# gpuopenanalytics/libgdf

Hardware: AMD Instinct MI355X
Metric: hash-join probe rows/s (higher is better)
Workload: dtype int64

## Files before the change

libgdf_amd/csrc/internal.h:

```cpp
#pragma once
#include "common.h"
#include "lab.h"
#include "prof.h"

namespace gdf_amd {

hipError_t read_back(void *host_dst, const void *dev_src, size_t bytes);
struct ReadTicket { bool pending = false; int lane = 0; size_t bytes = 0; const void *dev_src = nullptr; };
hipError_t read_back_begin(ReadTicket *t, const void *dev_src, size_t bytes, int lane);
hipError_t read_back_end(ReadTicket *t, void *host_dst);

void place_budget_begin();
bool place_budget_left();
int place_draws_now(int max_draws);
struct PlaceRound {
  double t0;
  PlaceRound();
  ~PlaceRound();
};

int device_cu_count();

gdf_error scan_u32(const uint32_t *in, uint32_t *out, size_t n, bool inclusive);
gdf_error scan_u64(const uint64_t *in, uint64_t *out, size_t n, bool inclusive);
gdf_error scan_u32_async(const uint32_t *in, uint32_t *out, size_t n, bool inclusive, DevBuf *scratch);

gdf_error order_rows(const KeyTable &t, uint32_t n, DevBuf &perm, DevBuf *sorted_keys, bool *keys_exact, size_t *perm64 = nullptr,
                     bool *perm64_written = nullptr);
gdf_error key_ranges(const KeyTable &t, long long *lo_hi, int windows = 1, int64_t window_rows = 0);
gdf_error radix_sort_pairs_u64(uint64_t *&kin, uint64_t *&kout, uint64_t *&vin, uint64_t *&vout, uint32_t n, uint64_t varying);
gdf_error radix_sort_pairs_k32_u64(uint32_t *&kin, uint32_t *&kout, uint64_t *&vin, uint64_t *&vout, uint32_t n, uint64_t varying);
gdf_error group_by_sort(int ncols, gdf_column **cols, gdf_column *col_agg, gdf_column *out_col_indices,
                        gdf_column **out_col_values, gdf_column *out_col_agg, gdf_context *ctxt, int op);

}
```

libgdf_amd/csrc/join.hip:

```cpp
#include "internal.h"
#include "launch.h"
#include "gdf/gdf_amd_ext.h"

#include <cmath>
#include <cstdio>

#include <algorithm>
#include <cstdlib>
#include <deque>
#include <memory>
#include <type_traits>
#include <vector>

namespace gdf_amd {

enum KeyMode : int { KM_RAW_INT = 0, KM_RAW_FLOAT, KM_PACKED, KM_HASHED };

struct KeyPlan {
  int mode;
  int verify;
  int narrow;
  uint64_t kmin;
  uint64_t kspan;
  uint64_t klimit;
// ... 1120 lines not shown
  const T incl = wave_scan_incl(v);
  block_sync();
  if (lane_id() == WAVE - 1) lds_wave[threadIdx.x / WAVE] = incl;
  block_sync();
  T woff = 0, tot = 0;
#pragma unroll
  for (int w = 0; w < JK_BK_THREADS / WAVE; ++w) {
    if (w < (int)(threadIdx.x / WAVE)) woff += lds_wave[w];
    tot += lds_wave[w];
  }
  *total = tot;
  return woff + incl - v;
}
constexpr uint32_t JK_L2MAP_LDS_SEGS = 16384;
__global__ __launch_bounds__(JK_BK_THREADS) void jk_make_l2map(const uint32_t *__restrict__ fill, uint32_t nseg, uint32_t cap1, uint32_t tile,
                                                               uint32_t *__restrict__ seg_begin, uint32_t *__restrict__ seg_end,
                                                               uint32_t *__restrict__ tile_prefix, uint32_t *__restrict__ ntiles,
                                                               uint32_t fj_world, uint32_t ncoarse, const uint32_t *__restrict__ rstart = nullptr,
                                                               const uint32_t *__restrict__ rcap = nullptr) {
  __shared__ uint32_t lds_wave[JK_BK_THREADS / WAVE];
  extern __shared__ __attribute__((aligned(16))) uint32_t l2map_lds[];
  const uint32_t per = (nseg + JK_BK_THREADS - 1) / JK_BK_THREADS;
  const uint32_t c0 = threadIdx.x * per;
  auto region_of = [&](uint32_t seg) -> uint32_t {
    if (!fj_world) return seg;
    const uint32_t cs = seg >> 3, c = cs / fj_world, sender = cs - c * fj_world;
    return ((sender * ncoarse + c) << 3) | (seg & 7u);
  };
  auto filled = [&](uint32_t region) -> uint32_t { const uint32_t n = fill[region], room = rcap ? rcap[region] : cap1; return n < room ? n : room; };
  const bool pow2 = (tile & (tile - 1u)) == 0;
  const int shift = __ffs((int)tile) - 1;
  auto tiles_of = [&](uint32_t n) -> uint32_t { return pow2 ? (n + tile - 1u) >> shift : (n + tile - 1u) / tile; };
  if (nseg <= JK_L2MAP_LDS_SEGS) {
    constexpr int MAXK = (int)(JK_L2MAP_LDS_SEGS / JK_BK_THREADS);
    uint32_t n_[MAXK], first_[MAXK];
#pragma unroll
    for (int k = 0; k < MAXK; ++k) {
      const uint32_t c = (uint32_t)k * JK_BK_THREADS + threadIdx.x;
      n_[k] = 0; first_[k] = 0;
      if (c < nseg) {
        const uint32_t r = region_of(c);
        n_[k] = filled(r);
        first_[k] = rstart ? rstart[r] : r * cap1;
        l2map_lds[c] = tiles_of(n_[k]);
      }
    }
    block_sync();
    uint32_t mine = 0;
    for (uint32_t c = c0; c < c0 + per && c < nseg; ++c) mine += l2map_lds[c];
    uint32_t total;
    uint32_t run = bk_block_scan<uint32_t>(mine, lds_wave, &total);
    for (uint32_t c = c0; c < c0 + per && c < nseg; ++c) { const uint32_t t = l2map_lds[c]; l2map_lds[c] = run; run += t; }
    block_sync();
#pragma unroll
    for (int k = 0; k < MAXK; ++k) {
      const uint32_t c = (uint32_t)k * JK_BK_THREADS + threadIdx.x;
      if (c < nseg) { seg_begin[c] = first_[k]; seg_end[c] = first_[k] + n_[k]; tile_prefix[c] = l2map_lds[c]; }
    }
    if (threadIdx.x == 0) { tile_prefix[nseg] = total; *ntiles = total; }
    return;
  }
  uint32_t mine = 0;
  for (uint32_t c = c0; c < c0 + per && c < nseg; ++c) mine += tiles_of(filled(region_of(c)));
  uint32_t total;
  uint32_t run = bk_block_scan<uint32_t>(mine, lds_wave, &total);
  for (uint32_t c = c0; c < c0 + per && c < nseg; ++c) {
    const uint32_t r = region_of(c), n = filled(r);
    const uint32_t first = rstart ? rstart[r] : r * cap1;
    seg_begin[c] = first;
    seg_end[c] = first + n;
    tile_prefix[c] = run;
    run += tiles_of(n);
  }
  if (threadIdx.x == 0) { tile_prefix[nseg] = total; *ntiles = total; }
}
static gdf_error l2map_prepare(uint32_t nseg, size_t *lds) {
  *lds = nseg <= JK_L2MAP_LDS_SEGS ? sizeof(uint32_t) * (size_t)nseg : 0;
  return allow_lds(jk_make_l2map, sizeof(uint32_t) * JK_L2MAP_LDS_SEGS);
}
__global__ __launch_bounds__(256) void jk_init_cursor(uint32_t *cur, uint32_t nfine, uint32_t cap2, const uint32_t *__restrict__ fstart = nullptr) {
  for (uint32_t f = blockIdx.x * 256 + threadIdx.x; f <= nfine; f += gridDim.x * 256) cur[f] = f < nfine ? (fstart ? fstart[f] : f * cap2) : 0u;
}

__global__ __launch_bounds__(JK_BK_THREADS) void jk_level2_index(const uint32_t *__restrict__ begin, const uint32_t *__restrict__ cnt, uint32_t nfine, int b2,
                                                                 uint32_t tile, uint32_t *__restrict__ coarse_off, uint32_t *__restrict__ tile_prefix,
                                                                 uint32_t *__restrict__ cursor) {
  __shared__ uint32_t lds_wave[JK_BK_THREADS / WAVE];
  const uint32_t ncoarse = nfine >> b2, total_rows = begin[nfine - 1] + cnt[nfine - 1];
  uint32_t run = 0;
  for (uint32_t base = 0; base < ncoarse; base += JK_BK_THREADS) {
    const uint32_t c = base + threadIdx.x;
    uint32_t first = 0, tiles = 0;
    if (c < ncoarse) {
      first = begin[(size_t)c << b2];
      const uint32_t next = c + 1 < ncoarse ? begin[(size_t)(c + 1) << b2] : total_rows;
      tiles = (next - first + tile - 1) / tile;
    }
    uint32_t total;
    const uint32_t before = bk_block_scan<uint32_t>(tiles, lds_wave, &total);
    if (c < ncoarse) { coarse_off[c] = first; tile_prefix[c] = run + before; }
    run += total;
    block_sync();
  }
  if (threadIdx.x == 0) { coarse_off[ncoarse] = total_rows; tile_prefix[ncoarse] = run; }
  for (uint32_t f = threadIdx.x; f < nfine; f += JK_BK_THREADS) cursor[f] = begin[f];
}

struct Unit {
  uint32_t build_begin, build_count;
  uint32_t probe_begin, probe_count;
};

__global__ __launch_bounds__(256) void jk_make_units(uint32_t nfine, uint32_t cap2, const uint32_t *__restrict__ cursor,
                                                     const uint32_t *__restrict__ level1_flag,
                                                     const uint32_t *__restrict__ build_begin, const uint32_t *__restrict__ build_cnt,
                                                     int keep_probe, Unit *__restrict__ units, uint64_t *__restrict__ off,
                                                     unsigned long long *__restrict__ state, const uint32_t *__restrict__ fstart = nullptr,
                                                     const uint32_t *__restrict__ fcap = nullptr) {
  const uint32_t f = blockIdx.x * 256 + threadIdx.x;
  const uint32_t fc = f < nfine ? f : nfine - 1;
  const uint32_t cur = cursor[fc], bn = build_cnt[fc], bb = build_begin[fc];
  const uint32_t first = fstart ? fstart[fc] : fc * cap2;
  if (fcap) cap2 = fcap[fc];
  const uint32_t grown = f < nfine ? cur - first : 0u;
  const uint32_t all = grown < cap2 ? grown : cap2;
  const uint32_t pn = (all != 0 && (bn != 0 || keep_probe)) ? all : 0u;
  const uint32_t nun = (pn + JK_PROBE_CHUNK - 1) / JK_PROBE_CHUNK;
  const uint32_t incl_u = wave_scan_incl(nun);
  const unsigned long long incl_t = wave_scan_incl((unsigned long long)pn);
  const unsigned long long sum_all = wave_reduce_add((unsigned long long)all);
  unsigned long long base_u = 0, base_t = 0;
  if (lane_id() == WAVE - 1) {
    if (incl_u) { base_u = atomicAdd(&state[0], (unsigned long long)incl_u); base_t = atomicAdd(&state[1], incl_t); }
    if (sum_all) atomicAdd(&state[2], sum_all);
  }
  base_u = __shfl(base_u, WAVE - 1, WAVE);
  base_t = __shfl(base_t, WAVE - 1, WAVE);
  unsigned long long u = base_u + incl_u - nun, o = base_t + incl_t - pn;
  for (uint32_t at = 0; at < pn; at += JK_PROBE_CHUNK) {
    const uint32_t cnt = pn - at < JK_PROBE_CHUNK ? pn - at : JK_PROBE_CHUNK;
    units[u] = Unit{bb, bn, first + at, cnt};
    off[u] = o;
    ++u;
    o += cnt;
  }
  if (f == 0) state[3] = (unsigned long long)((cursor[nfine] ? 1u : 0u) | ((level1_flag && *level1_flag) ? 2u : 0u));
}

struct ProbeArgs {
  Tuples build, probe;
  const Unit *units;
  uint32_t nslots;
  uint32_t cap;
  int keep_unmatched_probe;
  int verify;
  uint8_t *build_matched;
  uint64_t *counts;
  int32_t *out_probe; int32_t *out_build;
  int unused;
  uint64_t kbias;
  int optimistic;
  unsigned long long *opt_state;
  uint32_t *unit_todo;
  uint32_t sample_n;
  const unsigned long long *nunits_dev;
  uint32_t *unit_pairs;
  int pay_mode;
  const void *pay_src[2];
  void *pay_out[2];
  int key_width;
  const void *key_src;
  void *key_out;
  int bpay_mode;
  const void *bpay_src[2];
  void *bpay_out[2];
  int p6_fb;
  uint32_t p6_world;
  uint64_t p6_kbias;
};
__device__ __forceinline__ void pay_gather(const ProbeArgs &a, unsigned long long pos, int32_t prow) {
  if (a.pay_mode == 1 || a.pay_mode == 4) {
    ((uint64_t *)a.pay_out[0])[pos] = ((const uint64_t *)a.pay_src[0])[prow];
    if (a.pay_mode == 4) ((uint64_t *)a.pay_out[1])[pos] = ((const uint64_t *)a.pay_src[1])[prow];
  } else if (a.pay_mode) {
    ((uint32_t *)a.pay_out[0])[pos] = ((const uint32_t *)a.pay_src[0])[prow];
    if (a.pay_mode == 3) ((uint32_t *)a.pay_out[1])[pos] = ((const uint32_t *)a.pay_src[1])[prow];
  }
  if (a.key_width == 8) ((uint64_t *)a.key_out)[pos] = ((const uint64_t *)a.key_src)[prow];
// ... 1351 lines not shown
    } else {
      const size_t lds = sizeof(TileLds<true, 1024>);
      GDF_TRY(with_int<8, 4>(fast, [&](auto F) {
        return with_bools([&](auto M) {
          return launch_lds("jk_scatter1", jk_scatter1<F(), true, 1024, M(), true>, dim3(g.nchunks), dim3(1024), lds, t, plan, g, H1off, out);
        }, masked);
      }));
    }
    HIP_CHECK_LAST();
    return GDF_SUCCESS;
  }
  if (masked) {
    if (fast == 4) return launch_scatter1_n<4, true, true>(t, plan, g, H1off, out);
    return narrow ? launch_scatter1_n<8, true, true>(t, plan, g, H1off, out)
                  : launch_scatter1_n<8, false, true>(t, plan, g, H1off, out);
  }
  if (fast == 4) return launch_scatter1_n<4, true, false>(t, plan, g, H1off, out);
  if (fast == 8) return narrow ? launch_scatter1_n<8, true, false>(t, plan, g, H1off, out)
                               : launch_scatter1_n<8, false, false>(t, plan, g, H1off, out);
  return narrow ? launch_scatter1_n<0, true, false>(t, plan, g, H1off, out)
                : launch_scatter1_n<0, false, false>(t, plan, g, H1off, out);
}
static int fast_key_width(const KeyTable &t, const KeyPlan &plan) {
  if (t.ncols != 1 || (plan.mode != KM_RAW_INT && plan.mode != KM_RAW_FLOAT) || t.nrows < 2) return 0;
  if (t.col[0].valid && t.nrows < 64) return 0;
  if (t.col[0].width == 8) return 8;
  if (t.col[0].width == 4 && plan.narrow && plan.kmin == 0) return 4;
  return 0;
}
template <bool NARROW, int THREADS>
static constexpr size_t level2_lds_bytes() { using Tile = TileLds<NARROW, THREADS>; return offsetof(Tile, cursor); }
static gdf_error launch_scatter2(bool narrow, uint32_t ntiles, const PartGeom &g, Level2Map m, Tuples in,
                                 uint32_t *cursor, Tuples out, bool p6 = false, bool in6 = false, int pw = 1) {
  if (in6 && !(p6 && !m.keys32 && g.b1 == 8)) return GDF_INVALID_API_CALL;
  if (!in6 && p6 && !narrow && m.keys32) return GDF_INVALID_API_CALL;
  m.ntiles = ntiles;
  m.xcd_order = (ntiles >= 64 && !lab::path_on("GDF_JK_NO_XCD_ORDER")) ? 1 : 0;
  const uint32_t grid = sc2_grid(m, ntiles);
  auto launch = [&](const char *name, auto kernel, int threads, size_t lds) -> gdf_error {
    GDF_TRY(launch_lds(name, kernel, dim3(grid), dim3(threads), lds, g, m, in, cursor, out));
    HIP_CHECK_LAST();
    return GDF_SUCCESS;
  };
  if (in6) {
    if (!narrow)
      return launch("jk_scatter2_w10", jk_scatter2<false, 256, 0, true, false, true>, 256, level2_lds_bytes<false, 256>());
    return launch("jk_scatter2", jk_scatter2<true, 256, 0, true, false, true>, 256, sizeof(TileLds<true, 256>));
  }
  if (p6 && !narrow)
    return launch("jk_scatter2_w10", jk_scatter2<false, 256, 0, true>, 256, level2_lds_bytes<false, 256>());
  if (p6 || m.keys32) {
    const size_t lds = sizeof(TileLds<true, 256>);
    if (p6 && m.keys32) return launch("jk_scatter2", jk_scatter2<true, 256, 0, true, true>, 256, lds);
    if (p6) return launch("jk_scatter2", jk_scatter2<true, 256, 0, true, false>, 256, lds);
    return launch("jk_scatter2", jk_scatter2<true, 256, 0, false, true>, 256, lds);
  }
  if (narrow && in.pay && pw == 2) {
    using Tile = TileLds<true, 256, 2, JK_PAY_ITEMS>;
    return launch("jk_scatter2", jk_scatter2<true, 256, 2>, 256, offsetof(Tile, cursor));
  }
  if (narrow && in.pay)
    return launch("jk_scatter2", jk_scatter2<true, 256, 1>, 256, sizeof(TileLds<true, 256, true, JK_PAY_ITEMS>));
  if (narrow) return launch("jk_scatter2", jk_scatter2<true, JK_SC2_THREADS>, JK_SC2_THREADS, sizeof(TileLds<true, JK_SC2_THREADS>));
  return launch("jk_scatter2", jk_scatter2<false, JK_SC2_THREADS>, JK_SC2_THREADS, sizeof(TileLds<false, JK_SC2_THREADS>));
}

static gdf_error launch_scatter1_pay(int fast, int pmode, const KeyTable &t, const KeyPlan &plan, const PartGeom &g, const uint32_t *H1off,
                                     const PaySrc &ps, Tuples out) {
  GDF_TRY(with_int<8, 4>(fast, [&](auto F) {
    return with_int<1, 2, 3, 4>(pmode, [&](auto M) {
      const size_t lds = sizeof(TileLds<true, JK_PAY_THREADS, pay_words(M()), pay_items1(M())>);
      return launch_lds("jk_scatter1", jk_scatter1_pay<F(), M()>, dim3(g.nchunks), dim3(JK_PAY_THREADS), lds, t, plan, g, H1off, ps, out);
    });
  }));
  HIP_CHECK_LAST();
  return GDF_SUCCESS;
}

static gdf_error partition_side(const KeyTable &t, KeyPlan &plan, PartGeom g, SideBufs *sb, bool decide_narrow, const PaySrc *pay = nullptr,
                                int pmode = 0, bool device_index = false, bool want_p6 = false, bool keep_running = false) {
  const int64_t n = t.nrows;
  bool narrow = plan.narrow != 0;
  int64_t chunk = JK_CHUNK_ROWS;
  if (n / chunk > JK_MAX_CHUNKS) chunk = (n + JK_MAX_CHUNKS - 1) / JK_MAX_CHUNKS;
  constexpr int64_t MAX_TILE = 1024 * JK_SC_ITEMS;
  chunk = ((chunk + MAX_TILE - 1) / MAX_TILE) * MAX_TILE;
  g.chunk = chunk;
  g.nchunks = (int)((n + chunk - 1) / chunk);
  if (g.nchunks == 0) g.nchunks = 1;
  const uint32_t nfine = 1u << g.fb, ncoarse = 1u << g.b1;

  const int hist_grid = g.nchunks < NUM_CU ? g.nchunks : NUM_CU;
  const size_t hist_bytes = sizeof(uint32_t) * nfine + sizeof(long long) * 2 * (size_t)hist_grid;
  DevBuf fine_hist, H1;
  RMM_TRY(fine_hist.alloc(hist_bytes));
  RMM_TRY(H1.alloc(sizeof(uint32_t) * (size_t)ncoarse * g.nchunks));
  HIP_TRY(hipMemsetAsync(fine_hist.p, 0, sizeof(uint32_t) * nfine, stream0()));
  const size_t hist_lds = sizeof(uint32_t) * (nfine + ncoarse);
  const int fast = fast_key_width(t, plan);
  GDF_TRY(allow_lds(jk_hist<8>, hist_lds));
  GDF_TRY(allow_lds(jk_hist<4>, hist_lds));
  GDF_TRY(allow_lds(jk_hist<0>, hist_lds));
  long long *d_mm = nullptr;
  if (decide_narrow)
    d_mm = reinterpret_cast<long long *>(fine_hist.as<uint32_t>() + nfine);
  if (fast == 8)
    GDF_LAUNCH("jk_hist", jk_hist<8>, dim3(hist_grid), dim3(JK_HIST_THREADS), hist_lds, stream0(), t, plan, g,
               fine_hist.as<uint32_t>(), H1.as<uint32_t>(), d_mm);
  else if (fast == 4)
    GDF_LAUNCH("jk_hist", jk_hist<4>, dim3(hist_grid), dim3(JK_HIST_THREADS), hist_lds, stream0(), t, plan, g,
               fine_hist.as<uint32_t>(), H1.as<uint32_t>(), d_mm);
  else
    GDF_LAUNCH("jk_hist", jk_hist<0>, dim3(hist_grid), dim3(JK_HIST_THREADS), hist_lds, stream0(), t, plan, g,
               fine_hist.as<uint32_t>(), H1.as<uint32_t>(), d_mm);
  HIP_CHECK_LAST();
  std::vector<uint32_t> fh(hist_bytes / sizeof(uint32_t));
  ReadTicket hist_ticket;
  HIP_TRY(read_back_begin(&hist_ticket, fine_hist.p, d_mm ? hist_bytes : sizeof(uint32_t) * nfine, 0));
  DevBuf scan_a, scan_b, d_coarse, d_tiles, cursor;
  struct Quiesce { bool armed = true; ~Quiesce() { if (armed) (void)hipStreamSynchronize(stream0()); } } quiesce;
  GDF_TRY(scan_u32_async(H1.as<uint32_t>(), H1.as<uint32_t>(), (size_t)ncoarse * g.nchunks, false, &scan_a));
  if (device_index) {
    RMM_TRY(sb->d_begin.alloc(sizeof(uint32_t) * nfine));
    GDF_TRY(scan_u32_async(fine_hist.as<uint32_t>(), sb->d_begin.as<uint32_t>(), nfine, false, &scan_b));
  }
  HIP_TRY(read_back_end(&hist_ticket, fh.data()));
  long long h[2] = {LLONG_MAX, LLONG_MIN};
  if (d_mm) {
    const long long *wg = reinterpret_cast<const long long *>(fh.data() + nfine);
    for (int b = 0; b < hist_grid; ++b) { h[0] = std::min(h[0], wg[2 * b]); h[1] = std::max(h[1], wg[2 * b + 1]); }
  }
  fh.resize(nfine);
  sb->fine_off.assign(nfine + 1, 0);
  for (uint32_t f = 0; f < nfine; ++f) sb->fine_off[f + 1] = sb->fine_off[f] + fh[f];
  sb->joinable = sb->fine_off[nfine];
  sb->fine_begin.assign(sb->fine_off.begin(), sb->fine_off.begin() + nfine);
  sb->fine_cnt = fh;
  sb->speculative = false;
  if (device_index) {
    sb->d_cnt.reset();
    sb->d_cnt.p = fine_hist.release();
  }
  const size_t cap = sb->joinable ? sb->joinable : 1;
  if (d_mm) {
    if (h[0] <= h[1] && (uint64_t)h[1] - (uint64_t)h[0] < 0xffffffffULL) {
      plan.narrow = 1;
      plan.kmin = (uint64_t)h[0];
      plan.kspan = (uint64_t)h[1] - (uint64_t)h[0];
      plan.klimit = plan.kspan;
      plan.kwindow = (plan.kmin & 0xffffffffULL) + plan.kspan < (1ULL << 32) ? 0xffffffffULL - (plan.kmin & 0xffffffffULL) : 0xffffffffULL;
      narrow = true;
    }
  }
  g.kbias = plan.kmin;
  if (pay && !(narrow && fast && !t.col[0].valid)) pay = nullptr;
  const int64_t JK_TILE2 = (int64_t)JK_SC2_THREADS * (pay ? JK_PAY_ITEMS : JK_SC_ITEMS);

  g.dump = (uint32_t)(cap + 2);
  RMM_TRY(sb->w[0].alloc(sizeof(uint64_t) * (cap + 2 + 1024)));
  if (!narrow) RMM_TRY(sb->idx[0].alloc(sizeof(int32_t) * (cap + 2 + 1024)));
  const int pw = pay ? pay_words(pmode) : 1;
  sb->pay_words = pw;
  if (pay) RMM_TRY(sb->pay[0].alloc(sizeof(uint64_t) * pw * (cap + 2 + 1024)));
  const Tuples t0 = sb->tuples(0);
  const bool level2 = g.b2 > 0 && sb->joinable > 0;
  bool p6 = false;
  uint32_t ntiles = 0;
  std::vector<uint32_t> coarse_off, tile_prefix;
  if (level2) {
    coarse_off.resize(ncoarse + 1);
    tile_prefix.resize(ncoarse + 1);
    for (uint32_t c = 0; c <= ncoarse; ++c) coarse_off[c] = sb->fine_off[(size_t)c << g.b2];
    tile_prefix[0] = 0;
    for (uint32_t c = 0; c < ncoarse; ++c)
      tile_prefix[c + 1] = tile_prefix[c] + (coarse_off[c + 1] - coarse_off[c] + JK_TILE2 - 1) / JK_TILE2;
    ntiles = tile_prefix[ncoarse];
    RMM_TRY(d_coarse.alloc(sizeof(uint32_t) * (ncoarse + 1)));
    RMM_TRY(d_tiles.alloc(sizeof(uint32_t) * (ncoarse + 1)));
    RMM_TRY(cursor.alloc(sizeof(uint32_t) * nfine));
    if (device_index) {
      hipLaunchKernelGGL(jk_level2_index, dim3(1), dim3(JK_BK_THREADS), 0, stream0(), (const uint32_t *)sb->d_begin.as<uint32_t>(),
                         (const uint32_t *)sb->d_cnt.as<uint32_t>(), nfine, g.b2, (uint32_t)JK_TILE2, d_coarse.as<uint32_t>(), d_tiles.as<uint32_t>(),
                         cursor.as<uint32_t>());
      HIP_CHECK_LAST();
    } else {
      HIP_TRY(hipMemcpyAsync(d_coarse.p, coarse_off.data(), sizeof(uint32_t) * (ncoarse + 1), hipMemcpyHostToDevice, stream0()));
      HIP_TRY(hipMemcpyAsync(d_tiles.p, tile_prefix.data(), sizeof(uint32_t) * (ncoarse + 1), hipMemcpyHostToDevice, stream0()));
      HIP_TRY(hipMemcpyAsync(cursor.p, sb->fine_off.data(), sizeof(uint32_t) * nfine, hipMemcpyHostToDevice, stream0()));
    }
    p6 = want_p6 && !pay;
    RMM_TRY(sb->w[1].alloc(p6 ? 6 * (cap + 2) + 16 : sizeof(uint64_t) * (cap + 2)));
    if (!narrow) RMM_TRY(sb->idx[1].alloc(sizeof(int32_t) * (cap + 2)));
    if (pay) RMM_TRY(sb->pay[1].alloc(sizeof(uint64_t) * pw * (cap + 2)));
  }
  if (pay) GDF_TRY(launch_scatter1_pay(fast, pmode, t, plan, g, H1.as<uint32_t>(), *pay, t0));
  else GDF_TRY(launch_scatter1(fast, narrow, t, plan, g, H1.as<uint32_t>(), t0));
  HIP_CHECK_LAST();
  sb->final_buf = 0;
  if (level2) {
    Level2Map m{d_coarse.as<uint32_t>(), d_coarse.as<uint32_t>() + 1, d_tiles.as<uint32_t>()};
    if (ntiles) GDF_TRY(launch_scatter2(narrow, ntiles, g, m, sb->tuples(0), cursor.as<uint32_t>(), sb->tuples(1), p6, false, pw));
    HIP_CHECK_LAST();
    if (keep_running && device_index) {
      for (DevBuf *b : {&sb->w[0], &sb->idx[0], &sb->pay[0], &d_coarse, &d_tiles, &cursor, &H1, &fine_hist, &scan_a, &scan_b}) sb->keep(*b);
      quiesce.armed = false;
    } else {
      HIP_TRY(hipStreamSynchronize(stream0()));
      sb->w[0].reset();
      sb->idx[0].reset();
      sb->pay[0].reset();
    }
    sb->final_buf = 1;
    sb->p6 = p6;
  } else if (keep_running && device_index) {
    for (DevBuf *b : {&H1, &fine_hist, &scan_a, &scan_b}) sb->keep(*b);
    quiesce.armed = false;
  } else {
    HIP_TRY(hipStreamSynchronize(stream0()));
  }
  return GDF_SUCCESS;
}

struct SpecAppend {
  DevBuf cursor;
  uint32_t cap2 = 0;
  bool started = false;
  int64_t rows = 0;
};

static gdf_error partition_side_spec(const KeyTable &t, const KeyPlan &plan, PartGeom g, double dup, SideBufs *sb, bool *ok,
                                     SpecAppend *app = nullptr, bool defer = false, const PaySrc *pay = nullptr, int pmode = 0,
                                     bool want_p6 = false, const SkewCaps *caps = nullptr) {
  *ok = false;
  if (app) g.row_base = (int32_t)app->rows;
  const int64_t n = t.nrows;
  const bool narrow = plan.narrow != 0;
  int64_t chunk = JK_CHUNK_ROWS;
  if (n / chunk > JK_MAX_CHUNKS) chunk = (n + JK_MAX_CHUNKS - 1) / JK_MAX_CHUNKS;
  constexpr int64_t MAX_TILE = 1024 * JK_SC_ITEMS;
  chunk = ((chunk + MAX_TILE - 1) / MAX_TILE) * MAX_TILE;
  g.chunk = chunk;
  g.nchunks = (int)((n + chunk - 1) / chunk);
  if (g.nchunks == 0) g.nchunks = 1;
  const uint32_t nfine = 1u << g.fb, ncoarse = 1u << g.b1;
  const int fast = fast_key_width(t, plan);
  const bool w10 = want_p6 && defer && !app && !narrow && !pay && fast == 8 && g.b1 == 8 && g.b2 > 0 && chunk == ((int64_t)1 << 17) &&
                   n < (((int64_t)1 << 30) - ((int64_t)1 << 23)) && g.row_base == 0 &&
                   ((n >= ((int64_t)1 << 26) && !lab::path_on("GDF_JK_NO_XCD_SPLIT")) || lab::path_on("GDF_JK_FORCE_L6")) && !lab::path_on("GDF_JK_NO_L6");
  const int sc_threads = sc1_threads(narrow, fast);
  const int64_t JK_TILE = (int64_t)sc_threads * sc1_items(narrow, sc_threads);
  const int64_t JK_TILE2 = (int64_t)JK_SC2_THREADS * (pay ? JK_PAY_ITEMS : JK_SC_ITEMS);
  auto room = [dup](double mean, uint32_t align) {
    const double c = mean + 8.0 * std::sqrt(mean * (1.0 + dup)) + 64.0;
    return (uint32_t)(((uint64_t)c + align - 1) / align * align);
  };
  g.xs = (g.b2 > 0 && n >= ((int64_t)1 << 26) && !lab::path_on("GDF_JK_NO_XCD_SPLIT")) ? 3 : 0;
  const bool l6 = w10 || (want_p6 && defer && !app && narrow && !pay && fast != 0 && g.b1 == 8 && g.b2 > 0 &&
                          chunk == ((int64_t)1 << 17) && n < (((int64_t)1 << 30) - ((int64_t)1 << 23)) && g.row_base == 0 &&
                          (g.xs == 3 || lab::path_on("GDF_JK_FORCE_L6")) && !lab::path_on("GDF_JK_NO_L6"));
  if (l6) g.xs = 6;
  const uint32_t nseg = ncoarse << g.xs;
  uint32_t cap1 = room((double)n / nseg, 64), cap2 = app ? app->cap2 : (g.b2 ? room((double)n / nfine, 8) : 0);
  uint64_t size1 = (uint64_t)nseg * cap1 + JK_TILE, size2 = (uint64_t)nfine * cap2 + JK_TILE;
  std::vector<uint32_t> cap_words;
  if (caps) {
    if (!(defer && !app && g.b2 > 0 && !pay && caps->fine.size() == nfine)) return GDF_SUCCESS;
    cap_words.resize(2 * (size_t)nseg + 2 * (size_t)nfine);
    uint32_t *rstart = cap_words.data(), *rcap = rstart + nseg, *fstart = rcap + nseg, *fcap = fstart + nfine;
    const double scale = caps->rows_per_sample;
    uint64_t run1 = 0, run2 = 0;
    uint32_t max1 = 0, max2 = 0;
    const uint32_t nreg = 1u << g.xs;
    for (uint32_t c = 0; c < ncoarse; ++c) {
      double sc = 0;
      for (uint32_t f = c << g.b2; f < ((c + 1) << g.b2); ++f) {
        const double sf = (double)caps->fine[f];
        sc += sf;
        const double U = (sf + 6.0 * std::sqrt(sf + 1.0) + 4.0) * scale;
        const uint64_t cf = ((uint64_t)(U + 64.0) + 7) / 8 * 8;
        fstart[f] = (uint32_t)std::min<uint64_t>(run2, 0xffffffffULL);
        fcap[f] = (uint32_t)std::min<uint64_t>(cf, 0x7fffffffULL);
        run2 += cf;
        max2 = std::max(max2, fcap[f]);
      }
      const double Uc = (sc + 6.0 * std::sqrt(sc + 1.0) + 4.0) * scale / (double)nreg;
      const uint64_t cr = ((uint64_t)(Uc + 8.0 * std::sqrt(Uc) + 64.0) + 63) / 64 * 64;
      for (uint32_t r = 0; r < nreg; ++r) {
        rstart[c * nreg + r] = (uint32_t)std::min<uint64_t>(run1, 0xffffffffULL);
        rcap[c * nreg + r] = (uint32_t)std::min<uint64_t>(cr, 0x7fffffffULL);
        run1 += cr;
        max1 = std::max(max1, rcap[c * nreg + r]);
      }
    }
    size1 = run1 + JK_TILE;
    size2 = run2 + JK_TILE;
    cap1 = max1;
    cap2 = max2;
  }
  if (size1 >= 0x7fffffffULL || size2 >= 0x7fffffffULL) return GDF_SUCCESS;

// ... 2223 lines not shown
```

libgdf_amd/csrc/plumbing.cpp:

```cpp
#include "internal.h"

#include <cstdio>
#include <cstring>
#include <atomic>
#include <chrono>
#include <map>
#include <set>
#include <mutex>
#include <string>
#include <roctracer/roctx.h>

extern "C" __attribute__((weak, visibility("default"))) const char *gdf_amd_testhook_forced(const char *name);
extern "C" __attribute__((weak, visibility("default"))) void gdf_amd_testhook_note(const char *name, long long value);

namespace gdf_amd {

void note_hip_error(hipError_t e, const char *what, const char *file, int line) {
  std::fprintf(stderr, "ERROR: HIP runtime call %s in line %d of file %s failed with %s (%d).\n", what, line, file,
               hipGetErrorString(e), (int)e);
}

gdf_error make_key_table(gdf_column **cols, int ncols, KeyTable *out) {
  if (lab::path_on("GDF_FORCE_HOST_ALLOC_FAILURE")) throw std::bad_alloc();
  if (ncols > MAX_KEY_COLS) return GDF_JOIN_TOO_MANY_COLUMNS;
  out->ncols = ncols;
  out->any_valid = 0;
  out->nrows = ncols > 0 ? (int64_t)cols[0]->size : 0;
  for (int c = 0; c < ncols; ++c) {
    const ElemKind k = elem_kind(cols[c]->dtype);
    if (k == K_BAD) return GDF_UNSUPPORTED_DTYPE;
    out->col[c].data = cols[c]->data;
    out->col[c].valid = cols[c]->valid;
    out->col[c].kind = (int)k;
    out->col[c].width = kind_width(k);
    if (cols[c]->valid) out->any_valid = 1;
  }
  return GDF_SUCCESS;
}

int device_cu_count() {
  static thread_local int cached_dev = -1, cached = NUM_CU;
  int dev = 0;
  if (hipGetDevice(&dev) != hipSuccess) { (void)hipGetLastError(); return NUM_CU; }
  if (dev != cached_dev) {
    int n = 0;
    if (hipDeviceGetAttribute(&n, hipDeviceAttributeMultiprocessorCount, dev) == hipSuccess && n > 0) cached = n;
    else { (void)hipGetLastError(); cached = NUM_CU; }
    cached_dev = dev;
  }
  return cached;
}

hipError_t read_back(void *host_dst, const void *dev_src, size_t bytes) {
  static thread_local void *pinned = nullptr;
  static thread_local size_t capacity = 0;
  if (bytes == 0) return hipSuccess;
  if (bytes > capacity) {
    if (pinned) (void)hipHostFree(pinned);
    pinned = nullptr;
    capacity = 0;
    const size_t want = bytes < (1u << 20) ? (1u << 20) : bytes;
    hipError_t e = hipHostMalloc(&pinned, want, hipHostMallocPortable);
    if (e != hipSuccess) { pinned = nullptr; return hipMemcpy(host_dst, dev_src, bytes, hipMemcpyDeviceToHost); }
    capacity = want;
  }
  hipError_t e = hipMemcpyAsync(pinned, dev_src, bytes, hipMemcpyDeviceToHost, stream0());
  if (e != hipSuccess) return e;
  e = hipStreamSynchronize(stream0());
  if (e != hipSuccess) return e;
  std::memcpy(host_dst, pinned, bytes);
  return hipSuccess;
}

namespace {
struct ReadLane { void *pinned = nullptr; size_t capacity = 0; hipEvent_t ev = nullptr; };
thread_local ReadLane g_read_lane[2];
}
hipError_t read_back_begin(ReadTicket *t, const void *dev_src, size_t bytes, int lane) {
  ReadLane &l = g_read_lane[lane & 1];
  t->pending = false;
  t->lane = lane & 1;
  t->bytes = bytes;
  t->dev_src = dev_src;
  if (bytes == 0) return hipSuccess;
  if (!l.ev && hipEventCreateWithFlags(&l.ev, hipEventDisableTiming) != hipSuccess) { (void)hipGetLastError(); l.ev = nullptr; return hipSuccess; }
  if (bytes > l.capacity) {
    if (l.pinned) (void)hipHostFree(l.pinned);
    l.pinned = nullptr;
    l.capacity = 0;
    const size_t want = bytes < (1u << 18) ? (1u << 18) : bytes;
    if (hipHostMalloc(&l.pinned, want, hipHostMallocPortable) != hipSuccess) { (void)hipGetLastError(); l.pinned = nullptr; return hipSuccess; }
    l.capacity = want;
  }
  hipError_t e = hipMemcpyAsync(l.pinned, dev_src, bytes, hipMemcpyDeviceToHost, stream0());
  if (e != hipSuccess) return e;
  e = hipEventRecord(l.ev, stream0());
  if (e != hipSuccess) { (void)hipGetLastError(); return hipSuccess; }
  t->pending = true;
  return hipSuccess;
}
hipError_t read_back_end(ReadTicket *t, void *host_dst) {
  if (t->bytes == 0) return hipSuccess;
  if (!t->pending) return read_back(host_dst, t->dev_src, t->bytes);
  t->pending = false;
  ReadLane &l = g_read_lane[t->lane];
  const hipError_t e = hipEventSynchronize(l.ev);
  if (e != hipSuccess) return e;
  std::memcpy(host_dst, l.pinned, t->bytes);
  return hipSuccess;
}

namespace {
thread_local double g_place_spent_ms = 0.0, g_place_limit_ms = 0.0;
std::atomic<int> g_place_calls{0};
thread_local bool g_place_charged = false;
double now_ms() { return std::chrono::duration<double, std::milli>(std::chrono::steady_clock::now().time_since_epoch()).count(); }
}
void place_budget_begin() {
  g_place_spent_ms = 0.0;
  g_place_charged = false;
  g_place_limit_ms = g_place_calls.load(std::memory_order_relaxed) < 1 ? 6.0 : 24.0;
  if (const long long forced = lab::path_int("GDF_PLACE_BUDGET_MS", -1); forced >= 0) g_place_limit_ms = (double)forced;
}
bool place_budget_left() { return g_place_spent_ms < g_place_limit_ms; }
int place_draws_now(int max_draws) { return place_budget_left() ? max_draws : -1; }
PlaceRound::PlaceRound() : t0(now_ms()) {}
PlaceRound::~PlaceRound() {
  g_place_spent_ms += now_ms() - t0;
  if (!g_place_charged) { g_place_charged = true; g_place_calls.fetch_add(1, std::memory_order_relaxed); }
}

namespace lab {
const char *forced(const char *name) { return gdf_amd_testhook_forced ? gdf_amd_testhook_forced(name) : nullptr; }
void note(const char *name, long long value) { if (gdf_amd_testhook_note) gdf_amd_testhook_note(name, value); }
}

}

extern "C" {

gdf_size_type gdf_column_sizeof(void) { return sizeof(gdf_column); }

gdf_error gdf_column_view(gdf_column *column, void *data, gdf_valid_type *valid, gdf_size_type size,
                          gdf_dtype dtype) {
  column->data = data;
  column->valid = valid;
  column->size = size;
  column->dtype = dtype;
  column->null_count = 0;
  return GDF_SUCCESS;
}

gdf_error gdf_column_view_augmented(gdf_column *column, void *data, gdf_valid_type *valid, gdf_size_type size,
                                    gdf_dtype dtype, gdf_size_type null_count) {
  column->data = data;
  column->valid = valid;
  column->size = size;
  column->dtype = dtype;
  column->null_count = null_count;
  return GDF_SUCCESS;
}

gdf_error gdf_column_free(gdf_column *column) {
  RMM_TRY(rmmFree(column->data, (cudaStream_t)0));
  RMM_TRY(rmmFree(column->valid, (cudaStream_t)0));
  return GDF_SUCCESS;
}

gdf_error get_column_byte_width(gdf_column *col, int *width) {
  const int w = gdf_amd::dtype_width(col->dtype);
  *width = w;
  return w > 0 ? GDF_SUCCESS : GDF_UNSUPPORTED_DTYPE;
}

gdf_error gdf_context_view(gdf_context *context, int flag_sorted, gdf_method flag_method, int flag_distinct,
                           int flag_sort_result, int flag_sort_inplace) {
  context->flag_sorted = flag_sorted;
  context->flag_method = flag_method;
  context->flag_distinct = flag_distinct;
  context->flag_sort_result = flag_sort_result;
  context->flag_sort_inplace = flag_sort_inplace;
  return GDF_SUCCESS;
}
// ... 38 lines not shown
```

Measured before the change: 111.8 billion.

## Fuse partition layout scans into one device kernel and defer host index

```diff
diff --git a/libgdf_amd/csrc/internal.h b/libgdf_amd/csrc/internal.h
--- a/libgdf_amd/csrc/internal.h
+++ b/libgdf_amd/csrc/internal.h
@@ -9,6 +9,7 @@
 struct ReadTicket { bool pending = false; int lane = 0; size_t bytes = 0; const void *dev_src = nullptr; };
 hipError_t read_back_begin(ReadTicket *t, const void *dev_src, size_t bytes, int lane);
 hipError_t read_back_end(ReadTicket *t, void *host_dst);
+hipError_t read_back_peek(ReadTicket *t, size_t offset, size_t bytes, void *host_dst);
 
 void place_budget_begin();
 bool place_budget_left();
diff --git a/libgdf_amd/csrc/join.hip b/libgdf_amd/csrc/join.hip
--- a/libgdf_amd/csrc/join.hip
+++ b/libgdf_amd/csrc/join.hip
@@ -1226,11 +1226,91 @@
   for (uint32_t f = blockIdx.x * 256 + threadIdx.x; f <= nfine; f += gridDim.x * 256) cur[f] = f < nfine ? (fstart ? fstart[f] : f * cap2) : 0u;
 }
 
-__global__ __launch_bounds__(JK_BK_THREADS) void jk_level2_index(const uint32_t *__restrict__ begin, const uint32_t *__restrict__ cnt, uint32_t nfine, int b2,
-                                                                 uint32_t tile, uint32_t *__restrict__ coarse_off, uint32_t *__restrict__ tile_prefix,
-                                                                 uint32_t *__restrict__ cursor) {
+struct LayoutState {
+  long long kmin, kmax;
+  uint32_t joinable;
+  uint32_t ntiles;
+  uint32_t narrow;
+  uint32_t largest;
+};
+__device__ __forceinline__ bool narrow_range(long long lo, long long hi) { return lo <= hi && (uint64_t)hi - (uint64_t)lo < 0xffffffffULL; }
+__global__ __launch_bounds__(JK_BK_THREADS) void jk_layout(const uint32_t *__restrict__ fine_hist, uint32_t nfine, int b2, uint32_t *__restrict__ H1,
+                                                           uint32_t nchunks, uint32_t *begin, uint32_t *__restrict__ coarse_off,
+                                                           uint32_t *__restrict__ tile_prefix, uint32_t *__restrict__ cursor,
+                                                           const long long *__restrict__ minmax, uint32_t nminmax, int narrow_plan,
+                                                           uint32_t tile_narrow, uint32_t tile_wide, LayoutState *__restrict__ state) {
   __shared__ uint32_t lds_wave[JK_BK_THREADS / WAVE];
-  const uint32_t ncoarse = nfine >> b2, total_rows = begin[nfine - 1] + cnt[nfine - 1];
+  const uint32_t ncoarse = nfine >> b2;
+  if (blockIdx.x < ncoarse) {
+    const uint32_t in_front = blockIdx.x << b2;
+    uint32_t *row = H1 + (size_t)blockIdx.x * nchunks;
+    uint32_t v = threadIdx.x < nchunks ? row[threadIdx.x] : 0u;
+    uint32_t mine = 0;
+#pragma unroll 4
+    for (uint32_t f = threadIdx.x; f < in_front; f += JK_BK_THREADS) mine += fine_hist[f];
+    uint32_t run;
+    (void)bk_block_scan<uint32_t>(mine, lds_wave, &run);
+    for (uint32_t base = 0; base < nchunks; base += JK_BK_THREADS) {
+      const uint32_t k = base + threadIdx.x, next = k + JK_BK_THREADS;
+      const uint32_t v_next = next < nchunks ? row[next] : 0u;
+      uint32_t total;
+      const uint32_t before = bk_block_scan<uint32_t>(v, lds_wave, &total);
+      if (k < nchunks) row[k] = run + before;
+      run += total;
+      v = v_next;
+    }
+    return;
+  }
+  __shared__ long long wg_mm[2];
+  __shared__ uint32_t wg_largest;
+  if (threadIdx.x == 0) { wg_mm[0] = LLONG_MAX; wg_mm[1] = LLONG_MIN; wg_largest = 0; }
+  block_sync();
+  if (minmax && threadIdx.x < WAVE) {
+    long long lo = LLONG_MAX, hi = LLONG_MIN;
+    for (uint32_t b = threadIdx.x; b < nminmax; b += WAVE) {
+      const long long l2 = minmax[2 * b], h2 = minmax[2 * b + 1];
+      lo = l2 < lo ? l2 : lo;
+      hi = h2 > hi ? h2 : hi;
+    }
+    if (lo <= hi) { atomicMin(&wg_mm[0], lo); atomicMax(&wg_mm[1], hi); }
+  }
+  const uint32_t rows = (nfine + JK_BK_THREADS - 1) / JK_BK_THREADS;
+  const uint32_t wave_first = (threadIdx.x / WAVE) * rows * WAVE + (uint32_t)lane_id();
+  uint32_t lane_total = 0, largest = 0;
+#pragma unroll 4
+  for (uint32_t r = 0; r < rows; ++r) {
+    const uint32_t f = wave_first + r * WAVE;
+    const uint32_t v = f < nfine ? fine_hist[f] : 0u;
+    lane_total += v;
+    largest = v > largest ? v : largest;
+  }
+  if (largest) atomicMax(&wg_largest, largest);
+  const uint32_t wave_total = wave_reduce_add(lane_total);
+  uint32_t total_rows;
+  uint32_t run_f = bk_block_scan<uint32_t>(lane_id() == 0 ? wave_total : 0u, lds_wave, &total_rows);
+  run_f = __shfl(run_f, 0, WAVE);
+  constexpr uint32_t GROUP = 4;
+  for (uint32_t r0 = 0; r0 < rows; r0 += GROUP) {
+    uint32_t v[GROUP];
+#pragma unroll
+    for (uint32_t j = 0; j < GROUP; ++j) {
+      const uint32_t f = wave_first + (r0 + j) * WAVE;
+      v[j] = (r0 + j < rows && f < nfine) ? fine_hist[f] : 0u;
+    }
+#pragma unroll
+    for (uint32_t j = 0; j < GROUP; ++j) {
+      const uint32_t f = wave_first + (r0 + j) * WAVE;
+      const uint32_t incl = wave_scan_incl(v[j]);
+      if (r0 + j < rows && f < nfine) {
+        begin[f] = run_f + incl - v[j];
+        if (cursor) cursor[f] = run_f + incl - v[j];
+      }
+      run_f += __shfl(incl, WAVE - 1, WAVE);
+    }
+  }
+  block_sync();
+  const bool narrow = narrow_plan || narrow_range(wg_mm[0], wg_mm[1]);
+  const uint32_t tile = narrow ? tile_narrow : tile_wide;
   uint32_t run = 0;
   for (uint32_t base = 0; base < ncoarse; base += JK_BK_THREADS) {
     const uint32_t c = base + threadIdx.x;
@@ -1242,12 +1322,13 @@
     }
     uint32_t total;
     const uint32_t before = bk_block_scan<uint32_t>(tiles, lds_wave, &total);
-    if (c < ncoarse) { coarse_off[c] = first; tile_prefix[c] = run + before; }
+    if (coarse_off && c < ncoarse) { coarse_off[c] = first; tile_prefix[c] = run + before; }
     run += total;
-    block_sync();
-  }
-  if (threadIdx.x == 0) { coarse_off[ncoarse] = total_rows; tile_prefix[ncoarse] = run; }
-  for (uint32_t f = threadIdx.x; f < nfine; f += JK_BK_THREADS) cursor[f] = begin[f];
+  }
+  if (threadIdx.x == 0) {
+    if (coarse_off) { coarse_off[ncoarse] = total_rows; tile_prefix[ncoarse] = run; }
+    *state = LayoutState{wg_mm[0], wg_mm[1], total_rows, run, narrow ? 1u : 0u, wg_largest};
+  }
 }
 
 struct Unit {
@@ -2765,6 +2846,7 @@
   const int64_t n = t.nrows;
   bool narrow = plan.narrow != 0;
   int64_t chunk = JK_CHUNK_ROWS;
+  if (const long long forced = lab::path_int("GDF_JK_CHUNK_ROWS", 0); forced > 0) chunk = forced;
   if (n / chunk > JK_MAX_CHUNKS) chunk = (n + JK_MAX_CHUNKS - 1) / JK_MAX_CHUNKS;
   constexpr int64_t MAX_TILE = 1024 * JK_SC_ITEMS;
   chunk = ((chunk + MAX_TILE - 1) / MAX_TILE) * MAX_TILE;
@@ -2772,9 +2854,11 @@
   g.nchunks = (int)((n + chunk - 1) / chunk);
   if (g.nchunks == 0) g.nchunks = 1;
   const uint32_t nfine = 1u << g.fb, ncoarse = 1u << g.b1;
+  lab::note(device_index ? "jk_layout_index_chunks" : "jk_layout_chunks", g.nchunks);
 
   const int hist_grid = g.nchunks < NUM_CU ? g.nchunks : NUM_CU;
-  const size_t hist_bytes = sizeof(uint32_t) * nfine + sizeof(long long) * 2 * (size_t)hist_grid;
+  const size_t mm_at = (sizeof(uint32_t) * nfine + 7) & ~(size_t)7, state_at = mm_at + sizeof(long long) * 2 * (size_t)hist_grid;
+  const size_t hist_bytes = state_at + sizeof(LayoutState);
   DevBuf fine_hist, H1;
   RMM_TRY(fine_hist.alloc(hist_bytes));
   RMM_TRY(H1.alloc(sizeof(uint32_t) * (size_t)ncoarse * g.nchunks));
@@ -2786,7 +2870,7 @@
   GDF_TRY(allow_lds(jk_hist<0>, hist_lds));
   long long *d_mm = nullptr;
   if (decide_narrow)
-    d_mm = reinterpret_cast<long long *>(fine_hist.as<uint32_t>() + nfine);
+    d_mm = reinterpret_cast<long long *>(fine_hist.as<unsigned char>() + mm_at);
   if (fast == 8)
     GDF_LAUNCH("jk_hist", jk_hist<8>, dim3(hist_grid), dim3(JK_HIST_THREADS), hist_lds, stream0(), t, plan, g,
                fine_hist.as<uint32_t>(), H1.as<uint32_t>(), d_mm);
@@ -2799,31 +2883,49 @@
   HIP_CHECK_LAST();
   std::vector<uint32_t> fh(hist_bytes / sizeof(uint32_t));
   ReadTicket hist_ticket;
-  HIP_TRY(read_back_begin(&hist_ticket, fine_hist.p, d_mm ? hist_bytes : sizeof(uint32_t) * nfine, 0));
-  DevBuf scan_a, scan_b, d_coarse, d_tiles, cursor;
+  DevBuf d_coarse, d_tiles, cursor;
   struct Quiesce { bool armed = true; ~Quiesce() { if (armed) (void)hipStreamSynchronize(stream0()); } } quiesce;
-  GDF_TRY(scan_u32_async(H1.as<uint32_t>(), H1.as<uint32_t>(), (size_t)ncoarse * g.nchunks, false, &scan_a));
+  const uint32_t tile_plain = (uint32_t)JK_SC2_THREADS * JK_SC_ITEMS;
+  const uint32_t tile_pay = (pay && fast && !t.col[0].valid) ? (uint32_t)JK_SC2_THREADS * JK_PAY_ITEMS : tile_plain;
   if (device_index) {
     RMM_TRY(sb->d_begin.alloc(sizeof(uint32_t) * nfine));
-    GDF_TRY(scan_u32_async(fine_hist.as<uint32_t>(), sb->d_begin.as<uint32_t>(), nfine, false, &scan_b));
-  }
-  HIP_TRY(read_back_end(&hist_ticket, fh.data()));
-  long long h[2] = {LLONG_MAX, LLONG_MIN};
-  if (d_mm) {
-    const long long *wg = reinterpret_cast<const long long *>(fh.data() + nfine);
-    for (int b = 0; b < hist_grid; ++b) { h[0] = std::min(h[0], wg[2 * b]); h[1] = std::max(h[1], wg[2 * b + 1]); }
-  }
-  fh.resize(nfine);
-  sb->fine_off.assign(nfine + 1, 0);
-  for (uint32_t f = 0; f < nfine; ++f) sb->fine_off[f + 1] = sb->fine_off[f] + fh[f];
-  sb->joinable = sb->fine_off[nfine];
-  sb->fine_begin.assign(sb->fine_off.begin(), sb->fine_off.begin() + nfine);
-  sb->fine_cnt = fh;
-  sb->speculative = false;
+    if (g.b2 > 0) {
+      RMM_TRY(d_coarse.alloc(sizeof(uint32_t) * (ncoarse + 1)));
+      RMM_TRY(d_tiles.alloc(sizeof(uint32_t) * (ncoarse + 1)));
+      RMM_TRY(cursor.alloc(sizeof(uint32_t) * nfine));
+    }
+  }
+  GDF_LAUNCH("jk_layout", jk_layout, dim3(ncoarse + (device_index ? 1 : 0)), dim3(JK_BK_THREADS), 0, stream0(), (const uint32_t *)fine_hist.as<uint32_t>(),
+             nfine, g.b2, H1.as<uint32_t>(), (uint32_t)g.nchunks, device_index ? sb->d_begin.as<uint32_t>() : nullptr, d_coarse.as<uint32_t>(), d_tiles.as<uint32_t>(),
+             cursor.as<uint32_t>(), (const long long *)d_mm, (uint32_t)hist_grid, (int)narrow, tile_pay, tile_plain,
+             reinterpret_cast<LayoutState *>(fine_hist.as<unsigned char>() + state_at));
+  HIP_CHECK_LAST();
+  HIP_TRY(read_back_begin(&hist_ticket, fine_hist.p, device_index ? hist_bytes : d_mm ? state_at : sizeof(uint32_t) * nfine, 0));
+  LayoutState ls{LLONG_MAX, LLONG_MIN, 0, 0, 0, 0};
+  auto host_index = [&]() -> gdf_error {
+    HIP_TRY(read_back_end(&hist_ticket, fh.data()));
+    if (d_mm && !device_index) {
+      const long long *wg = reinterpret_cast<const long long *>(reinterpret_cast<const unsigned char *>(fh.data()) + mm_at);
+      for (int b = 0; b < hist_grid; ++b) { ls.kmin = std::min(ls.kmin, wg[2 * b]); ls.kmax = std::max(ls.kmax, wg[2 * b + 1]); }
+    }
+    fh.resize(nfine);
+    sb->fine_off.assign(nfine + 1, 0);
+    for (uint32_t f = 0; f < nfine; ++f) sb->fine_off[f + 1] = sb->fine_off[f] + fh[f];
+    sb->fine_begin.assign(sb->fine_off.begin(), sb->fine_off.begin() + nfine);
+    sb->fine_cnt = fh;
+    return GDF_SUCCESS;
+  };
   if (device_index) {
+    HIP_TRY(read_back_peek(&hist_ticket, state_at, sizeof(ls), &ls));
+    sb->joinable = ls.joinable;
     sb->d_cnt.reset();
     sb->d_cnt.p = fine_hist.release();
-  }
+  } else {
+    GDF_TRY(host_index());
+    sb->joinable = sb->fine_off[nfine];
+  }
+  const long long h[2] = {ls.kmin, ls.kmax};
+  sb->speculative = false;
   const size_t cap = sb->joinable ? sb->joinable : 1;
   if (d_mm) {
     if (h[0] <= h[1] && (uint64_t)h[1] - (uint64_t)h[0] < 0xffffffffULL) {
@@ -2851,22 +2953,19 @@
   uint32_t ntiles = 0;
   std::vector<uint32_t> coarse_off, tile_prefix;
   if (level2) {
-    coarse_off.resize(ncoarse + 1);
-    tile_prefix.resize(ncoarse + 1);
-    for (uint32_t c = 0; c <= ncoarse; ++c) coarse_off[c] = sb->fine_off[(size_t)c << g.b2];
-    tile_prefix[0] = 0;
-    for (uint32_t c = 0; c < ncoarse; ++c)
-      tile_prefix[c + 1] = tile_prefix[c] + (coarse_off[c + 1] - coarse_off[c] + JK_TILE2 - 1) / JK_TILE2;
-    ntiles = tile_prefix[ncoarse];
-    RMM_TRY(d_coarse.alloc(sizeof(uint32_t) * (ncoarse + 1)));
-    RMM_TRY(d_tiles.alloc(sizeof(uint32_t) * (ncoarse + 1)));
-    RMM_TRY(cursor.alloc(sizeof(uint32_t) * nfine));
     if (device_index) {
-      hipLaunchKernelGGL(jk_level2_index, dim3(1), dim3(JK_BK_THREADS), 0, stream0(), (const uint32_t *)sb->d_begin.as<uint32_t>(),
-                         (const uint32_t *)sb->d_cnt.as<uint32_t>(), nfine, g.b2, (uint32_t)JK_TILE2, d_coarse.as<uint32_t>(), d_tiles.as<uint32_t>(),
-                         cursor.as<uint32_t>());
-      HIP_CHECK_LAST();
+      ntiles = ls.ntiles;
     } else {
+      coarse_off.resize(ncoarse + 1);
+      tile_prefix.resize(ncoarse + 1);
+      for (uint32_t c = 0; c <= ncoarse; ++c) coarse_off[c] = sb->fine_off[(size_t)c << g.b2];
+      tile_prefix[0] = 0;
+      for (uint32_t c = 0; c < ncoarse; ++c)
+        tile_prefix[c + 1] = tile_prefix[c] + (coarse_off[c + 1] - coarse_off[c] + JK_TILE2 - 1) / JK_TILE2;
+      ntiles = tile_prefix[ncoarse];
+      RMM_TRY(d_coarse.alloc(sizeof(uint32_t) * (ncoarse + 1)));
+      RMM_TRY(d_tiles.alloc(sizeof(uint32_t) * (ncoarse + 1)));
+      RMM_TRY(cursor.alloc(sizeof(uint32_t) * nfine));
       HIP_TRY(hipMemcpyAsync(d_coarse.p, coarse_off.data(), sizeof(uint32_t) * (ncoarse + 1), hipMemcpyHostToDevice, stream0()));
       HIP_TRY(hipMemcpyAsync(d_tiles.p, tile_prefix.data(), sizeof(uint32_t) * (ncoarse + 1), hipMemcpyHostToDevice, stream0()));
       HIP_TRY(hipMemcpyAsync(cursor.p, sb->fine_off.data(), sizeof(uint32_t) * nfine, hipMemcpyHostToDevice, stream0()));
@@ -2884,8 +2983,9 @@
     Level2Map m{d_coarse.as<uint32_t>(), d_coarse.as<uint32_t>() + 1, d_tiles.as<uint32_t>()};
     if (ntiles) GDF_TRY(launch_scatter2(narrow, ntiles, g, m, sb->tuples(0), cursor.as<uint32_t>(), sb->tuples(1), p6, false, pw));
     HIP_CHECK_LAST();
+    if (device_index) GDF_TRY(host_index());
     if (keep_running && device_index) {
-      for (DevBuf *b : {&sb->w[0], &sb->idx[0], &sb->pay[0], &d_coarse, &d_tiles, &cursor, &H1, &fine_hist, &scan_a, &scan_b}) sb->keep(*b);
+      for (DevBuf *b : {&sb->w[0], &sb->idx[0], &sb->pay[0], &d_coarse, &d_tiles, &cursor, &H1, &fine_hist}) sb->keep(*b);
       quiesce.armed = false;
     } else {
       HIP_TRY(hipStreamSynchronize(stream0()));
@@ -2896,9 +2996,11 @@
     sb->final_buf = 1;
     sb->p6 = p6;
   } else if (keep_running && device_index) {
-    for (DevBuf *b : {&H1, &fine_hist, &scan_a, &scan_b}) sb->keep(*b);
+    GDF_TRY(host_index());
+    for (DevBuf *b : {&H1, &fine_hist, &d_coarse, &d_tiles, &cursor}) sb->keep(*b);
     quiesce.armed = false;
   } else {
+    if (device_index) GDF_TRY(host_index());
     HIP_TRY(hipStreamSynchronize(stream0()));
   }
   return GDF_SUCCESS;
diff --git a/libgdf_amd/csrc/plumbing.cpp b/libgdf_amd/csrc/plumbing.cpp
--- a/libgdf_amd/csrc/plumbing.cpp
+++ b/libgdf_amd/csrc/plumbing.cpp
@@ -99,6 +99,15 @@
   t->pending = true;
   return hipSuccess;
 }
+hipError_t read_back_peek(ReadTicket *t, size_t offset, size_t bytes, void *host_dst) {
+  if (bytes == 0) return hipSuccess;
+  if (!t->pending) return read_back(host_dst, static_cast<const char *>(t->dev_src) + offset, bytes);
+  ReadLane &l = g_read_lane[t->lane];
+  const hipError_t e = hipEventSynchronize(l.ev);
+  if (e != hipSuccess) return e;
+  std::memcpy(host_dst, static_cast<const char *>(l.pinned) + offset, bytes);
+  return hipSuccess;
+}
 hipError_t read_back_end(ReadTicket *t, void *host_dst) {
   if (t->bytes == 0) return hipSuccess;
   if (!t->pending) return read_back(host_dst, t->dev_src, t->bytes);
```

Measured after the change: 101.9 billion. 0.911x the previous value.
